# lastdancewithyou/multimodal_edema_prediction

Measured on AMD Instinct MI355X. Metric: multimodal train samples/sec, higher is better.
Workload: dtype bf16

## Files before the change

### include/medp_hip.h

```cpp
#ifndef MEDP_HIP_H
#define MEDP_HIP_H
#include <stddef.h>

#ifdef __cplusplus
extern "C" {
#endif

const char* medp_last_error(void);
int medp_version(void);
const char* medp_arch(void);

int medp_gemm_bf16_nt(const void* A, const void* W, void* C, int M, int N, int K, int lda, int ldw, int ldc,
                      const float* bias, const float* scale, const float* residual, int ldr, int act, int out_bf16,
                      void* stream);

size_t medp_gemm_nt_workspace_bytes(int M, int N, int K);
int medp_gemm_bf16_nt_ws(const void* A, const void* W, void* C, int M, int N, int K, int lda, int ldw, int ldc, const float* bias,
                         const float* scale, const float* residual, int ldr, int act, int out_bf16, float* workspace,
                         size_t workspace_bytes, void* stream);

int medp_gemm_f32_nt(const float* A, const float* W, float* C, int M, int N, int K, int lda, int ldw, int ldc, const float* bias,
                     const float* scale, const float* residual, int ldr, int act, void* stream);
int medp_gemm_f32_tn(const float* dY, const float* X, float* C, int M, int N, int K, int lddy, int ldx, void* stream);

// ... 65 lines not shown

int medp_cast_f32_bf16(const float* x, int ldx, void* y, int ldy, int rows, int cols, void* stream);
int medp_transpose_to_bf16(const void* x, int x_is_bf16, int ldx, void* y, int ldy, int rows, int cols, void* stream);
typedef struct {
    const void* src;
    void* dst_plain;
    void* dst_t;
    int rows, cols, ld_src, ld_plain, ld_t, reserved_;
} MedpOperandJob;
int medp_weight_operands_multi(const MedpOperandJob* dev_jobs, const int* dev_block_job, const int* dev_block_tile, int n_blocks,
                               void* stream);
int medp_gelu_bwd(const float* dy, const float* pre, float* dx, long long n, void* stream);
int medp_gelu_bf16_fwd(const void* pre, void* out, long long n, void* stream);
int medp_gelu_bf16_bwd(const void* dy, const void* pre, void* dx, long long n, void* stream);
int medp_im2col_patch(const float* pix, void* A, int B, int C, int H, int W, int patch, int kpad, void* stream);
int medp_vit_assemble(const float* patch, const float* cls, const float* pos, float* x, int B, int P, int D, void* stream);
int medp_pos_embed_bicubic(const float* pos, float* out, int src_side, int gh, int gw, int D, void* stream);
int medp_pos_embed_bicubic_bwd(const float* dout, float* dpos, int src_side, int gh, int gw, int D, void* stream);

typedef struct {
    const float *ln1_w, *ln1_b;
    const void* qkv_w;
    const float* qkv_b;
    const void* proj_w;
    const float *proj_b, *ls1;
    const float *ln2_w, *ln2_b;
    const void* fc1_w;
    const float* fc1_b;
    const void* fc2_w;
    const float *fc2_b, *ls2;
    const void *qkv_wg, *fc1_wg;
    const float *qkv_cs, *qkv_b2, *fc1_cs, *fc1_b2;
} MedpVitLayer;

typedef struct {
    int hidden, n_layers, n_heads, mlp_hidden, patch, pos_side, patch_kpad;
    float ln_eps;
    const void* patch_w;
    const float *patch_b, *cls, *pos;
    const float *final_ln_w, *final_ln_b;
    const MedpVitLayer* layers;
} MedpVitWeights;

size_t medp_vit_workspace_bytes(const MedpVitWeights* host_w, int B, int H, int W);
int medp_vit_forward(const MedpVitWeights* host_w, const float* pixels, int B, int H, int W, float* tokens_f32,
                     void* tokens_bf16, void* workspace, size_t workspace_bytes, void* stream);
int medp_vit_forward_part(const MedpVitWeights* w, const float* pixels, int B, int H, int W, float* tokens_f32, void* tokens_bf16,
                          void* workspace, size_t workspace_bytes, int first_layer, int last_layer, void* stream);

typedef struct {
    const float* g_attn;
    const void* qkv_w;
    const void* out_w;
    const float* g_ff;
    const void* ff1_w;
    const float* ff1_b;
    const void* ff2_w;
    const float* ff2_b;
    const float* g_final;
} MedpEncoderWeights;

typedef struct {
    int n_vars, n_static, d_embedding, n_heads, n_layers, d_ff, d_hidden_embed, d_hidden_tab, d_hidden_time, n_obs_rows,
// ... 193 lines not shown
```

### multimodal_edema_prediction_amd/abi.py

```python
from __future__ import annotations

import ctypes
import os
from ctypes import c_char_p, c_double, c_float, c_int, c_longlong, c_size_t, c_uint, c_void_p

import numpy as np
import torch

_HERE = os.path.dirname(os.path.abspath(__file__))
LIB_PATH = os.environ.get("MEDP_HIP_LIB") or os.path.join(_HERE, "libmedp_hip.so")

P, I, F, U, LL, SZ = c_void_p, c_int, c_float, c_uint, c_longlong, c_size_t


class MedpVitLayer(ctypes.Structure):
    _fields_ = [(n, P) for n in ("ln1_w", "ln1_b", "qkv_w", "qkv_b", "proj_w", "proj_b", "ls1", "ln2_w", "ln2_b",
                                 "fc1_w", "fc1_b", "fc2_w", "fc2_b", "ls2",
                                 "qkv_wg", "fc1_wg", "qkv_cs", "qkv_b2", "fc1_cs", "fc1_b2")]


class MedpVitWeights(ctypes.Structure):
    _fields_ = ([(n, I) for n in ("hidden", "n_layers", "n_heads", "mlp_hidden", "patch", "pos_side", "patch_kpad")]
                + [("ln_eps", F)]
                + [(n, P) for n in ("patch_w", "patch_b", "cls", "pos", "final_ln_w", "final_ln_b")]
                + [("layers", ctypes.POINTER(MedpVitLayer))])


class MedpEncoderWeights(ctypes.Structure):
    _fields_ = [(n, P) for n in ("g_attn", "qkv_w", "out_w", "g_ff", "ff1_w", "ff1_b", "ff2_w", "ff2_b", "g_final")]


class MedpDuettWeights(ctypes.Structure):
    _fields_ = ([(n, I) for n in ("n_vars", "n_static", "d_embedding", "n_heads", "n_layers", "d_ff", "d_hidden_embed",
                                  "d_hidden_tab", "d_hidden_time", "n_obs_rows", "final_norm")]
                + [("norm_eps", F)]
                + [(n, P) for n in ("emb_b4", "emb_l0", "emb_w4t", "n_obs_table",
                                    "tab_w0", "tab_b0", "tab_bn_scale", "tab_bn_shift", "tab_w4", "tab_b4", "special",
                                    "time_w0", "time_b0", "time_bn_scale", "time_bn_shift", "time_w3t", "time_b3",
                                    "rep_embedding", "event_embedding")]
                + [("event_enc", ctypes.POINTER(MedpEncoderWeights)), ("time_enc", ctypes.POINTER(MedpEncoderWeights))])


class MedpAdamTensor(ctypes.Structure):
    _fields_ = [("param", P), ("grad", P), ("exp_avg", P), ("exp_avg_sq", P), ("numel", LL), ("lr", F), ("weight_decay", F)]


class MedpOperandJob(ctypes.Structure):
    _fields_ = [("src", P), ("dst_plain", P), ("dst_t", P), ("rows", I), ("cols", I), ("ld_src", I), ("ld_plain", I), ("ld_t", I),
                ("reserved_", I)]


class MedpProbeProblem(ctypes.Structure):
    _fields_ = [("col_off", LL), ("row_off", LL), ("n_rows", I), ("F", I), ("y_col", I), ("j0", I), ("j1", I), ("reserved_", I)]


class MedpHeadProblem(ctypes.Structure):
    _fields_ = ([(n, P) for n in ("X", "Y", "M", "W", "b", "mW", "vW", "mb", "vb", "t", "perm", "loss_out")] + [("ldx", LL)]
                + [(n, I) for n in ("N", "ldy", "col0", "F", "L", "label_width", "bs", "S")]
                + [(n, c_double) for n in ("lr", "weight_decay", "beta1", "beta2", "eps")]
                + [("dropout_p", F), ("seed", U), ("stream_id", U), ("reserved_", I)])


SIGNATURES = {
    "medp_last_error": (c_char_p, []),
# ... 26 lines not shown
    "medp_attn_fq_split_bwd": (I, [P, I, P, I, P, P, I, LL, P, P, I, LL, P, I, P, P, I, LL, P, SZ, I, I, I, I, I, F, F, U, U, P]),
    "medp_layernorm_fwd": (I, [P, I, P, P, P, I, I, P, P, I, I, F, P]),
    "medp_colsum_workspace_bytes": (SZ, [I, I]),
    "medp_layernorm_bwd": (I, [P, I, P, I, P, P, P, P, I, I, P, P, P, I, I, P]),
    "medp_colsum_f32": (I, [P, I, P, P, I, I, P]),
    "medp_scalenorm_fwd": (I, [P, I, P, P, I, I, P, I, I, F, P]),
    "medp_scalenorm_bwd": (I, [P, I, P, I, P, P, P, I, I, P, P, I, I, P]),
    "medp_scalenorm_bwd_add": (I, [P, I, P, I, P, P, P, I, P, I, P, P, I, I, P]),
    "medp_cast_f32_bf16": (I, [P, I, P, I, I, I, P]),
    "medp_transpose_to_bf16": (I, [P, I, I, P, I, I, I, P]),
    "medp_weight_operands_multi": (I, [P, P, P, I, P]),
    "medp_gelu_bwd": (I, [P, P, P, LL, P]),
    "medp_gelu_bf16_fwd": (I, [P, P, LL, P]),
    "medp_gelu_bf16_bwd": (I, [P, P, P, LL, P]),
    "medp_im2col_patch": (I, [P, P, I, I, I, I, I, I, P]),
    "medp_vit_assemble": (I, [P, P, P, P, I, I, I, P]),
    "medp_pos_embed_bicubic": (I, [P, P, I, I, I, I, P]),
    "medp_pos_embed_bicubic_bwd": (I, [P, P, I, I, I, I, P]),
    "medp_vit_workspace_bytes": (SZ, [ctypes.POINTER(MedpVitWeights), I, I, I]),
    "medp_vit_forward": (I, [ctypes.POINTER(MedpVitWeights), P, I, I, I, P, P, P, SZ, P]),
    "medp_vit_forward_part": (I, [ctypes.POINTER(MedpVitWeights), P, I, I, I, P, P, P, SZ, I, I, P]),
    "medp_duett_embed_fwd": (I, [ctypes.POINTER(MedpDuettWeights), P, P, P, I, I, P, P, P, P, P, I, P]),
    "medp_duett_swap_add_norm": (I, [P, P, P, P, LL, P, F, P, P, I, I, I, I, P]),
    "medp_feats_to_input": (I, [P, P, LL, P, P, LL, P, I, P, P, P, P, I, I, I, I, I, F, F, U, U, P]),
    "medp_ssl_mask_batch": (I, [P, P, P, P, P, P, P, P, P, I, I, I, P]),
    "medp_duett_workspace_bytes": (SZ, [ctypes.POINTER(MedpDuettWeights), I, I]),
    "medp_duett_encode": (I, [ctypes.POINTER(MedpDuettWeights), P, P, P, I, I, P, P, P, P, SZ, P]),
    "medp_gelu_dropout_fwd": (I, [P, P, LL, F, U, U, P]),
    "medp_gelu_dropout_bwd": (I, [P, P, P, LL, F, U, U, P]),
    "medp_gelu_dropout_fwd_bf16": (I, [P, P, LL, F, U, U, P]),
    "medp_gelu_dropout_bwd_bf16": (I, [P, P, P, P, LL, F, U, U, P]),
    "medp_dropout_add": (I, [P, P, P, LL, F, U, U, P]),
    "medp_rowdot_fwd": (I, [P, I, P, P, P, I, I, P]),
    "medp_rowdot_bwd": (I, [P, P, I, P, P, P, P, I, I, P]),
    "medp_fusion_logits_fwd": (I, [P, P, P, P, P, P, P, P, P, P, I, I, P]),
    "medp_fusion_logits_bwd": (I, [P, P, P, P, P, P, P, P, P, P, P, P, I, I, P]),
# ... 110 lines not shown
```

### multimodal_edema_prediction_amd/csrc/elementwise.hip

```cpp
#include "common.h"
#include "medp_hip.h"

namespace {

__global__ __launch_bounds__(256) void cast_f32_bf16_kernel(const float* __restrict__ x, int ldx, bf16_t* __restrict__ y, int ldy,
                                                            int rows, int cols) {
    const int c4 = cols >> 2;
    const size_t total = (size_t)rows * c4;
    for (size_t i = (size_t)blockIdx.x * 256 + threadIdx.x; i < total; i += (size_t)gridDim.x * 256) {
        const int r = (int)(i / c4), c = (int)(i % c4) * 4;
        const float4 v = *(const float4*)(x + (size_t)r * ldx + c);
        uint2 o;
        o.x = pack_bf2(v.x, v.y);
        o.y = pack_bf2(v.z, v.w);
        *(uint2*)(y + (size_t)r * ldy + c) = o;
    }
}

template <typename TIN>
__global__ __launch_bounds__(256) void transpose_to_bf16_kernel(const TIN* __restrict__ x, int ldx, bf16_t* __restrict__ y, int ldy,
                                                                int rows, int cols) {
    __shared__ float tile[64][65];
    const int r0 = blockIdx.y * 64, c0 = blockIdx.x * 64;
    const int tx = threadIdx.x & 63, ty = threadIdx.x >> 6;
// ... 67 lines not shown
                                                            bf16_t* __restrict__ dx, size_t n8) {
    for (size_t i = (size_t)blockIdx.x * 256 + threadIdx.x; i < n8; i += (size_t)gridDim.x * 256) {
        const uint4 g = *(const uint4*)(dy + i * 8), p = *(const uint4*)(pre + i * 8);
        const uint32_t gw[4] = {g.x, g.y, g.z, g.w}, pw[4] = {p.x, p.y, p.z, p.w};
        uint32_t o[4];
#pragma unroll
        for (int k = 0; k < 4; ++k) {
            const float a = __uint_as_float(gw[k] << 16) * gelu_erf_grad(__uint_as_float(pw[k] << 16));
            const float b = __uint_as_float(gw[k] & 0xffff0000u) * gelu_erf_grad(__uint_as_float(pw[k] & 0xffff0000u));
            o[k] = pack_bf2(a, b);
        }
        *(uint4*)(dx + i * 8) = make_uint4(o[0], o[1], o[2], o[3]);
    }
}

__global__ __launch_bounds__(256) void im2col_patch_kernel(const float* __restrict__ pix, bf16_t* __restrict__ A, int B, int C, int H,
                                                           int W, int ps, int kpad) {
    const unsigned gh = H / ps, gw = W / ps, K = C * ps * ps, pp = ps * ps, k8 = kpad >> 3;
    const unsigned total = (unsigned)B * gh * gw * k8;
    for (unsigned i = blockIdx.x * 256u + threadIdx.x; i < total; i += gridDim.x * 256u) {
        const unsigned kc = i % k8, row = i / k8;
        const unsigned px = row % gw, r2 = row / gw, py = r2 % gh, b = r2 / gh;
        const float* img = pix + (size_t)b * C * H * W + (size_t)(py * ps) * W + px * ps;
        float v[8];
#pragma unroll
        for (int u = 0; u < 8; ++u) {
            const unsigned kk = kc * 8 + u;
            float x = 0.f;
            if (kk < K) {
                const unsigned c = kk / pp, rem = kk - c * pp, ii = rem / ps, jj = rem - ii * ps;
                x = img[((size_t)c * H + ii) * W + jj];
            }
// ... 133 lines not shown
extern "C" int medp_gelu_bf16_fwd(const void* pre, void* out, long long n, void* stream) {
    MEDP_CHECK_ARG(pre && out && n > 0 && n % 8 == 0, "gelu_bf16_fwd: bad argument (n must be a multiple of 8)");
    gelu_bf16_fwd_kernel<<<grid_for((size_t)n / 8), 256, 0, (hipStream_t)stream>>>((const bf16_t*)pre, (bf16_t*)out, (size_t)n / 8);
    MEDP_LAUNCH_CHECK("medp_gelu_bf16_fwd");
    return 0;
}

extern "C" int medp_gelu_bf16_bwd(const void* dy, const void* pre, void* dx, long long n, void* stream) {
    MEDP_CHECK_ARG(dy && pre && dx && n > 0 && n % 8 == 0, "gelu_bf16_bwd: bad argument (n must be a multiple of 8)");
    gelu_bf16_bwd_kernel<<<grid_for((size_t)n / 8), 256, 0, (hipStream_t)stream>>>((const bf16_t*)dy, (const bf16_t*)pre, (bf16_t*)dx,
                                                                                  (size_t)n / 8);
    MEDP_LAUNCH_CHECK("medp_gelu_bf16_bwd");
    return 0;
}

extern "C" int medp_im2col_patch(const float* pix, void* A, int B, int C, int H, int W, int patch, int kpad, void* stream) {
    MEDP_CHECK_ARG(pix && A && B > 0 && C > 0 && patch > 0, "im2col: bad argument");
    MEDP_CHECK_ARG(H >= patch && W >= patch, "im2col: image %dx%d smaller than the patch size %d", H, W, patch);
    MEDP_CHECK_ARG(kpad >= C * patch * patch && kpad % 8 == 0, "im2col: kpad must be >= C*p*p and a multiple of 8");
    const size_t total = (size_t)B * (H / patch) * (W / patch) * (kpad / 8);
    MEDP_CHECK_ARG(total < (1ull << 31), "im2col: B * patches * kpad / 8 must stay below 2^31");
    im2col_patch_kernel<<<grid_for(total), 256, 0, (hipStream_t)stream>>>(pix, (bf16_t*)A, B, C, H, W, patch, kpad);
    MEDP_LAUNCH_CHECK("medp_im2col_patch");
    return 0;
}

extern "C" int medp_vit_assemble(const float* patch, const float* cls, const float* pos, float* x, int B, int P, int D, void* stream) {
    MEDP_CHECK_ARG(patch && cls && pos && x && B > 0 && P > 0 && D % 4 == 0, "vit_assemble: bad argument");
    vit_assemble_kernel<<<grid_for((size_t)B * (P + 1) * D / 4), 256, 0, (hipStream_t)stream>>>(patch, cls, pos, x, B, P, D);
    MEDP_LAUNCH_CHECK("medp_vit_assemble");
    return 0;
}

extern "C" int medp_pos_embed_bicubic_bwd(const float* dout, float* dpos, int src_side, int gh, int gw, int D, void* stream) {
    MEDP_CHECK_ARG(dout && dpos && src_side > 0 && gh > 0 && gw > 0 && D > 0 && D % 4 == 0, "pos_embed_bicubic_bwd: bad argument");
    pos_bicubic_bwd_kernel<<<grid_for((size_t)(src_side * src_side + 1) * (D / 4)), 256, 0, (hipStream_t)stream>>>(dout, dpos, src_side, gh, gw, D);
    MEDP_LAUNCH_CHECK("medp_pos_embed_bicubic_bwd");
    return 0;
// ... 9 lines not shown
```

### multimodal_edema_prediction_amd/csrc/vit.hip

```cpp
#include "common.h"
#include "gemm_variants.h"
#include "medp_hip.h"

namespace {
inline size_t al(size_t x) { return (x + 255) & ~(size_t)255; }

struct VitWs {
    size_t a0, patch, pos, x, h, qkv, att, f, xb, stats, total;
};

template <int NT>
__global__ __launch_bounds__(256) void rowstats_cast_kernel(const float* __restrict__ x, bf16_t* __restrict__ xb, float* __restrict__ stats,
                                                            int M, int Mpad, int D) {
    const int lane = threadIdx.x & 63;
    const int row = blockIdx.x * 4 + (threadIdx.x >> 6);
    if (row >= Mpad) return;
    float s1[NT], s2[NT];
#pragma unroll
    for (int k = 0; k < NT; ++k) {
        s1[k] = s2[k] = 0.f;
        if (row < M) {
            const float4 v = *(const float4*)(x + (size_t)row * D + 4 * (lane + 64 * k));
            uint2 o;
            o.x = pack_bf2(v.x, v.y);
// ... 45 lines not shown
    return medp_gemm_run(MedpGemmArgs{A, W, C, M, N, K, K, K, N, bias, scale, residual, N, act, out_bf16, nullptr, 0, fold}, 1, nullptr, 0, stream);
}
}

extern "C" size_t medp_vit_workspace_bytes(const MedpVitWeights* w, int B, int H, int W) {
    if (!w || B <= 0 || H <= 0 || W <= 0 || w->patch <= 0) return 0;
    return plan(w, B, H, W).total;
}

extern "C" int medp_vit_forward(const MedpVitWeights* w, const float* pixels, int B, int H, int W, float* tokens_f32,
                                void* tokens_bf16, void* workspace, size_t workspace_bytes, void* stream) {
    MEDP_CHECK_ARG(w, "vit_forward: null argument");
    return medp_vit_forward_part(w, pixels, B, H, W, tokens_f32, tokens_bf16, workspace, workspace_bytes, 0, w->n_layers, stream);
}

extern "C" int medp_vit_forward_part(const MedpVitWeights* w, const float* pixels, int B, int H, int W, float* tokens_f32,
                                     void* tokens_bf16, void* workspace, size_t workspace_bytes, int first_layer, int last_layer,
                                     void* stream) {
    MEDP_CHECK_ARG(w && pixels && workspace, "vit_forward: null argument");
    MEDP_CHECK_ARG(0 <= first_layer && first_layer <= last_layer && last_layer <= w->n_layers,
                   "vit_forward: bad layer range [%d, %d) of %d", first_layer, last_layer, w->n_layers);
    const bool embed = first_layer == 0, finish = last_layer == w->n_layers;
    MEDP_CHECK_ARG(!finish || tokens_f32 || tokens_bf16, "vit_forward: no output requested");
    MEDP_CHECK_ARG(w->hidden == w->n_heads * 64, "vit_forward: head dim must be 64 (hidden %d, heads %d)", w->hidden, w->n_heads);
    MEDP_CHECK_ARG(H >= w->patch && W >= w->patch, "vit_forward: image %dx%d smaller than one patch (%d)", H, W, w->patch);
    const VitWs ws = plan(w, B, H, W);
    MEDP_CHECK_ARG(workspace_bytes >= ws.total, "vit_forward: workspace %zu < required %zu", workspace_bytes, ws.total);
    char* base = (char*)workspace;
    const int gh = H / w->patch, gw = W / w->patch, P = gh * gw, S = P + 1, M = B * S, D = w->hidden;
    void* a0 = base + ws.a0;
    float* patch = (float*)(base + ws.patch);
    float* pos = (float*)(base + ws.pos);
    float* x = (float*)(base + ws.x);
    void* h = base + ws.h;
    void* qkv = base + ws.qkv;
    void* att = base + ws.att;
    void* f = base + ws.f;

    if (embed) {
        MEDP_TRY(medp_im2col_patch(pixels, a0, B, 3, H, W, w->patch, w->patch_kpad, stream));
        MEDP_TRY(medp_gemm_bf16_nt(a0, w->patch_w, patch, B * P, D, w->patch_kpad, w->patch_kpad, w->patch_kpad, D, w->patch_b,
                                   nullptr, nullptr, 0, 0, 0, stream));
        const float* pos_used = w->pos;
        if (!(gh == w->pos_side && gw == w->pos_side)) {
            MEDP_TRY(medp_pos_embed_bicubic(w->pos, pos, w->pos_side, gh, gw, D, stream));
            pos_used = pos;
        }
        MEDP_TRY(medp_vit_assemble(patch, w->cls, pos_used, x, B, P, D, stream));
    }
    const float scale = 0.125f;
    if (fold_wanted(w, M) && first_layer < last_layer) {
        bf16_t* xb = (bf16_t*)(base + ws.xb);
        float* stats = (float*)(base + ws.stats);
        const int NT = D / 256, Mpad = (M + 255) / 256 * 256;
        hipStream_t st = (hipStream_t)stream;
        if (NT == 1) rowstats_cast_kernel<1><<<(Mpad + 3) / 4, 256, 0, st>>>(x, xb, stats, M, Mpad, D);
        else if (NT == 2) rowstats_cast_kernel<2><<<(Mpad + 3) / 4, 256, 0, st>>>(x, xb, stats, M, Mpad, D);
        else if (NT == 3) rowstats_cast_kernel<3><<<(Mpad + 3) / 4, 256, 0, st>>>(x, xb, stats, M, Mpad, D);
        else rowstats_cast_kernel<4><<<(Mpad + 3) / 4, 256, 0, st>>>(x, xb, stats, M, Mpad, D);
        MEDP_LAUNCH_CHECK("vit rowstats_cast");
        MedpGemmFold cons{}, prod{};
// ... 19 lines not shown
            MEDP_TRY(medp_attn_fwd_dh64(qkv, (const bf16_t*)qkv + D, (const bf16_t*)qkv + 2 * D, att, B, S, w->n_heads, 3 * D, 3 * D,
                                        3 * D, D, scale, stream));
            MEDP_TRY(block_gemm(att, L.proj_w, x, M, D, D, L.proj_b, L.ls1, x, 0, 0, plain, stream));
            MEDP_TRY(medp_layernorm_fwd(x, D, L.ln2_w, L.ln2_b, h, D, 1, nullptr, nullptr, M, D, w->ln_eps, stream));
            MEDP_TRY(block_gemm(h, L.fc1_w, f, M, w->mlp_hidden, D, L.fc1_b, nullptr, nullptr, 1, 1, plain, stream));
            MEDP_TRY(block_gemm(f, L.fc2_w, x, M, D, w->mlp_hidden, L.fc2_b, L.ls2, x, 0, 0, plain, stream));
        }
    }
    if (!finish) return 0;
    if (tokens_f32)
        MEDP_TRY(medp_layernorm_fwd(x, D, w->final_ln_w, w->final_ln_b, tokens_f32, D, 0, nullptr, nullptr, M, D, w->ln_eps, stream));
    if (tokens_bf16)
        MEDP_TRY(medp_layernorm_fwd(x, D, w->final_ln_w, w->final_ln_b, tokens_bf16, D, 1, nullptr, nullptr, M, D, w->ln_eps, stream));
    return 0;
}

extern "C" int medp_dbg_vit_lnfold(int on) {
    const int prev = g_vit_lnfold;
    g_vit_lnfold = on < 0 ? -1 : (on != 0);
    return prev;
}

extern "C" int medp_dbg_gemm_fold(const void* A, const void* W, void* C, int M, int N, int K, const float* bias, const float* scale,
                                  const float* residual, int act, int out_bf16, void* c2, float* stats_out, const float* stats_in,
                                  int stats_tiles, const float* colsum, float ln_eps, int ln_dim, void* stream) {
    MedpGemmFold f{};
    f.c2 = c2; f.ldc2 = N; f.stats_out = stats_out;
    f.stats_in = stats_in; f.stats_tiles = stats_tiles; f.colsum = colsum; f.ln_eps = ln_eps; f.ln_dim = ln_dim;
    MEDP_CHECK_ARG(medp_gemm_fold_eligible(M, N, K), "gemm(fold): M=%d N=%d K=%d does not take the 256-tile kernels", M, N, K);
    return block_gemm(A, W, C, M, N, K, bias, scale, residual, act, out_bf16, f, stream);
// ... 2 lines not shown
```

### multimodal_edema_prediction_amd/cxr.py

```python
from __future__ import annotations

import ctypes
from collections import namedtuple
from dataclasses import dataclass

import torch
import torch.nn as nn

from . import abi
from . import functional as Fn
from .abi import MedpVitLayer, MedpVitWeights, check, lib, ptr, stream


@dataclass
class Dinov2Cfg:
    hidden_size: int = 768
    num_hidden_layers: int = 12
    num_attention_heads: int = 12
    mlp_ratio: int = 4
    patch_size: int = 14
    image_size: int = 518
    layer_norm_eps: float = 1e-6
    layerscale_value: float = 1.0
    num_channels: int = 3
# ... 117 lines not shown
            for name, W, b, g, beta in (("qkv", qkv_w, qkv_b, blk.ln1_w, blk.ln1_b), ("fc1", blk.w1, blk.b1, blk.ln2_w, blk.ln2_b)):
                W32 = W.detach().to(torch.float32)
                wg = bf(W32 * g.detach().to(torch.float32)[None, :])
                setattr(L, name + "_wg", ptr(wg))
                setattr(L, name + "_cs", ptr(f32(wg.to(torch.float32).sum(dim=1))))
                setattr(L, name + "_b2", ptr(f32(b.detach().to(torch.float32) + W32 @ beta.detach().to(torch.float32))))
        w = MedpVitWeights()
        w.hidden, w.n_layers, w.n_heads, w.mlp_hidden = D, c.num_hidden_layers, c.num_attention_heads, D * c.mlp_ratio
        w.patch, w.pos_side, w.patch_kpad, w.ln_eps = c.patch_size, c.image_size // c.patch_size, pw.shape[1], c.layer_norm_eps
        w.patch_w = ptr(bf(pw))
        w.patch_b = ptr(f32(sd["embeddings.patch_embeddings.projection.bias"]))
        w.cls = ptr(f32(sd["embeddings.cls_token"].reshape(-1)))
        w.pos = ptr(f32(sd["embeddings.position_embeddings"].reshape(-1, D)))
        w.final_ln_w, w.final_ln_b = ptr(f32(sd["layernorm.weight"])), ptr(f32(sd["layernorm.bias"]))
        w.layers = ctypes.cast(layers, ctypes.POINTER(MedpVitLayer))
        self._prep, self._prep_key = (w, layers, keep), key
        return self._prep

    def forward(self, pixel_values: torch.Tensor, want_f32: bool = True, want_bf16: bool = False, layers=None, slot: int = 0, out16=None):
        abi.require_gpu()
        if pixel_values.dim() != 4 or pixel_values.shape[1] != self.cfg.num_channels:
            raise ValueError("Make sure that the channel dimension of the pixel values match with the one set in the "
                             f"configuration. Expected {self.cfg.num_channels} but got {tuple(pixel_values.shape)}.")
        if any(p.requires_grad for p in self.parameters()) and torch.is_grad_enabled():
            from .cxr_train import forward_training
            if out16 is not None:
                raise ValueError("out16 is a frozen-path argument (the training path returns fp32 tokens with a gradient)")
            tok = forward_training(self, pixel_values)
            return (tok if want_f32 else None), (tok if want_bf16 else None)
        if Fn.precision() == "fp32" and layers is None:
            from .cxr_train import forward_fp32
            tok = forward_fp32(self, pixel_values)
            t16 = None
            if want_bf16:
                t16 = tok.to(torch.bfloat16) if out16 is None else out16.copy_(tok)
            return (tok if want_f32 else None), t16
        w, _, _ = self._prepare()
        px = pixel_values.detach().to(torch.float32).contiguous()
        B, _, H, W = px.shape
        P = (H // self.cfg.patch_size) * (W // self.cfg.patch_size)
        need = lib().medp_vit_workspace_bytes(ctypes.byref(w), B, H, W)
        ws = self._ws.get(slot)
        if ws is None or ws.numel() < need or ws.device != px.device:
            ws = self._ws[slot] = torch.empty(need, dtype=torch.uint8, device=px.device)
        D = self.cfg.hidden_size
        first, last = (0, self.cfg.num_hidden_layers) if layers is None else layers
        fin = last == self.cfg.num_hidden_layers
        out32 = torch.empty((B, P + 1, D), dtype=torch.float32, device=px.device) if (want_f32 and fin) else None
        if out16 is not None:
            if out16.shape != (B, P + 1, D) or out16.dtype != torch.bfloat16 or not out16.is_contiguous() or out16.device != px.device:
                raise ValueError("out16 must be a contiguous bf16 [B, P+1, hidden] tensor on the input's device")
        else:
            out16 = torch.empty((B, P + 1, D), dtype=torch.bfloat16, device=px.device) if (want_bf16 and fin) else None
        check(lib().medp_vit_forward_part(ctypes.byref(w), ptr(px), B, H, W, ptr(out32), ptr(out16), ptr(ws), need, first, last,
                                          stream()), "vit_forward")
        return out32, out16


class CXREncoder(nn.Module):

    def __init__(self, model_name: str = "microsoft/rad-dino", freeze: bool = True, return_patches: bool = True, *,
                 config: Dinov2Cfg | None = None):
        super().__init__()
        self.backbone = Dinov2Backbone(config)
        if config is None and model_name and model_name != "synthetic":
            self._try_load_pretrained(model_name)
        self.d_out = self.backbone.cfg.hidden_size
        self.return_patches = return_patches
        if freeze:
            for p in self.backbone.parameters():
# ... 18 lines not shown
        return self

    def forward(self, pixel_values: torch.Tensor):
        tokens, _ = self.backbone(pixel_values)
        cls = tokens[:, 0]
        if self.return_patches:
            return cls, tokens[:, 1:]
        return cls

    def forward_bf16(self, pixel_values: torch.Tensor, slot: int = 0, out=None):
        if Fn.precision() == "fp32" and out is None and not (any(p.requires_grad for p in self.backbone.parameters()) and torch.is_grad_enabled()):
            return self.backbone(pixel_values, want_f32=True, want_bf16=False)[0]
        _, t16 = self.backbone(pixel_values, want_f32=False, want_bf16=True, slot=slot, out16=out)
        return t16

    def forward_bf16_part(self, pixel_values: torch.Tensor, first: int, last: int):
        if any(p.requires_grad for p in self.backbone.parameters()):
            raise RuntimeError("the encoder can only be run in pieces when it is frozen")
        _, t16 = self.backbone(pixel_values, want_f32=False, want_bf16=True, layers=(first, last))
        return t16
```

### multimodal_edema_prediction_amd/graph_step.py

```python
from __future__ import annotations

import os

import torch

from . import autograd_ops as _A, dp, engine
from .streams import new_stream, note_capture_origin
from .abi import check, lib, ptr, stream


def _stacked(v):
    return v if torch.is_tensor(v) else torch.stack(tuple(v))


class _TrainSnapshot:

    def __init__(self, modules, epoch, params=(), optimizer=None, extra=()):
        self.params, self.opt, self.modules, self.epoch = list(params), optimizer, list(modules), epoch
        with torch.no_grad():
            self.p = [q.detach().clone() for q in self.params]
            self.bufs = [(m, n, b.detach().clone()) for m in self.modules for n, b in m.named_buffers()]
            self.extra = [(t, t.detach().clone()) for t in extra]
            self.epoch0 = epoch.detach().clone()
            if optimizer is not None:
                self.state = {id(q): {k: (v.detach().clone() if torch.is_tensor(v) else v) for k, v in optimizer.state.get(q, {}).items()}
                              for q in self.params}
                self.host_step = optimizer._step
# ... 102 lines not shown

    def _replay(self):
        self._check_frozen_unchanged()
        self.opt.refresh_lrs()
        self.g.replay()
        self._after_replay()
        return self.out

    def _after_replay(self):
        self.opt.note_external_step()


class _PipelinedStep(_CapturedStep):

    def _setup(self, optimizer, device, world, group, split, pipeline, warmup, before_capture, after_capture=None):
        self.world, self.group = world, group
        self.pipeline = bool(pipeline)
        self.split = bool(split) or world > 1
        self.arena = None
        self.force_collective = False
        self._pool = None
        self._expect = None
        self._staged, self.stage = None, None
        self.frozen_stream = new_stream(device) if self.pipeline else None
        self._build(optimizer, device, warmup, before_capture)
        if after_capture is not None:
            after_capture()
        self.phase_log = None
        if self.pipeline and os.environ.get("MEDP_PHASE_CHECK", "0") == "1":
            penalty, t_copy = self._staging_penalty()
            self.phase_log = (len(self._pad_streams), round(penalty * 1e3, 3), round(t_copy * 1e3, 3))

    def _streams_before_capture(self):
        self._pad_streams = [new_stream(self.device, raw=True) for _ in range(int(os.environ.get("MEDP_PRE_CAPTURE_STREAMS", str(self._default_pad_streams()))))]
        self.copy_stream = new_stream(self.device)

    def _default_pad_streams(self) -> int:
        return 3
# ... 5 lines not shown
            self.arena = dp.FlatGradArena(self.params, used=used, group=self.group)
            self.arena.bind(zero=True)
            snap.restore()
        self._zero_grads()
        self._advance()
        if last and os.environ.get("MEDP_OPERAND_POOL", "1") == "1":
            with _A.record_operands() as log:
                self._whole_fwd_bwd()
            self._pool = _A.WeightOperandPool(log, self.device)
        else:
            self._whole_fwd_bwd()
        self._allreduce()
        self.opt.step()

    def _captured_step(self):
        if not self.split:
            self._advance()
            return self._whole_fwd_bwd(then=self.opt.step)
        self.arena.flat.zero_()
        self._advance()
        return self._whole_fwd_bwd()

    def _staging_penalty(self, n: int = 6):
        import time
        dev_b, host_b = self._calib_batches()
        snap = _TrainSnapshot(self._stateful_modules(), self.epoch, self.params, self.opt, extra=self._handover_tensors())
        expect = self._expect

        def timed(pool, staged):
            ts = []
# ... 28 lines not shown
    def _zero_grads(self):
        if self.arena is None:
            self.opt.zero_grad(set_to_none=True)
        else:
            self.arena.bind(zero=True)

    def _advance(self):
        self._advance_epoch()
        if self._pool is not None:
            self._pool.refresh()

    def _allreduce(self):
        if self.arena is not None and (self.world > 1 or self.force_collective):
            self.arena.all_reduce(force=self.force_collective)

    def _whole_fwd_bwd(self, then=None):
        if not self.pipeline:
            out = self._train_fwd_bwd()
            if then is not None:
                then()
            return out
        cur = torch.cuda.current_stream(self.device)
        self.frozen_stream.wait_stream(cur)
        with torch.cuda.stream(self.frozen_stream):
            self._frozen_forward()
        out = self._train_fwd_bwd()
        if then is not None:
            then()
        cur.wait_stream(self.frozen_stream)
        self._hand_over()
        return out

    def _after_replay(self):
        if not self.split:
            return super()._after_replay()
        ring = self._split_events()
        ring[0].record()
        self._allreduce()
        ring[1].record()
        self.opt.relaunch()
# ... 21 lines not shown
        if self.stage is None:
            self.stage = {k: torch.empty_like(v) for k, v in self._stage_buffers().items()}
            self.h2d_done, self.stage_free = torch.cuda.Event(), torch.cuda.Event()
            self.stage_free.record(torch.cuda.current_stream(self.device))
        with torch.cuda.stream(self.copy_stream):
            self.copy_stream.wait_event(self.stage_free)
            self._stage_h2d(next_batch, after_next)
            self.h2d_done.record(self.copy_stream)
        self._staged = (next_batch, after_next)

    def step(self, batch: dict | None = None, next_batch: dict | None = None, after_next: dict | None = None) -> dict:
        st = self._staged
        staged = self.pipeline and batch is not None and next_batch is not None and st is not None and st[0] is batch and st[1] is next_batch
        if batch is not None and self.pipeline and self._expect is not batch:
            self.prime(batch)
        if staged:
            cur = torch.cuda.current_stream(self.device)
            cur.wait_event(self.h2d_done)
            self._take_staged()
            self.stage_free.record(cur)
            self._expect = next_batch
        else:
            if batch is not None:
                self.load_batch(batch)
            nb = next_batch if next_batch is not None else batch
            if self.pipeline and nb is not None:
                self._load_next(nb)
                self._expect = nb
        if self.pipeline and after_next is not None and next_batch is not None and not next_batch["pixel_values"].is_cuda:
            self._stage(next_batch, after_next)
        else:
            self._staged = None
        return self._replay()


class GraphedTeacherStep(_PipelinedStep):
    def __init__(self, teacher, loss_fn, optimizer, example_batch: dict, device, world: int = 1, group=None, warmup: int = 3,
                 split: bool = False, before_capture=None, pipeline_cxr: bool = False, after_capture=None):
        self.teacher, self.loss_fn = teacher, loss_fn
        b = engine._move_lists(example_batch, device)
        self.x_ts = torch.stack(b["x_ts"]).contiguous()
        self.x_static = torch.stack(b["x_static"]).contiguous()
        self.bin_ends = torch.stack(b["bin_ends"]).contiguous()
        self.pixels = b["pixel_values"].clone()
        if pipeline_cxr:
            if any(p.requires_grad for p in teacher.cxr.parameters()):
                raise ValueError("pipeline_cxr needs a frozen CXR encoder")
            self.pixels_next = self.pixels.clone()
            with torch.no_grad():
                self.tok_cur = teacher.cxr.forward_bf16(self.pixels).clone()
            self.tok_next = torch.empty_like(self.tok_cur)
        self.y_multi = b["y_multi"].clone().float()
        self.y_mask = b["y_multi_mask"].clone().float()
        engine._set_train_with_frozen_eval(teacher)
        self._setup(optimizer, device, world, group, split, pipeline_cxr, warmup, before_capture, after_capture)

    def _frozen_forward(self):
        with torch.no_grad():
            self.teacher.cxr.forward_bf16(self.pixels_next, out=self.tok_next)

    def _stateful_modules(self):
        return [self.teacher]

    def _handover_tensors(self):
        return [self.tok_cur] if self.pipeline else []

    def _small_buffers(self):
        return {"x_ts": self.x_ts, "x_static": self.x_static, "bin_ends": self.bin_ends, "y_multi": self.y_multi, "y_multi_mask": self.y_mask}

    def _calib_batches(self):
        d = {k: v.clone() for k, v in dict(self._small_buffers(), pixel_values=self.pixels).items()}
        h = {k: v.cpu().pin_memory() for k, v in d.items()}
        return [dict(d), dict(d)], [dict(h), dict(h)]

    def _hand_over(self):
        self.tok_cur.copy_(self.tok_next)

    def _train_fwd_bwd(self):
        B = self.x_ts.shape[0]
        out = self.teacher(tuple(self.x_ts[i] for i in range(B)), tuple(self.x_static[i] for i in range(B)),
                           tuple(self.bin_ends[i] for i in range(B)), self.pixels,
                           **({"_cxr_tokens16": self.tok_cur} if self.pipeline else {}))
        losses = self.loss_fn(out["img_logits"], out["ts_logits"], out["fusion_logits"], self.y_multi, self.y_mask)
        losses["total"].backward()
        return {"loss": losses["total"].detach(), "img_total": losses["img_total"], "ts_total": losses["ts_total"],
                "fus_total": losses["fus_total"], "fusion_logits": out["fusion_logits"].detach(), "main_logit": out["main_logit"].detach()}

    def prime(self, batch: dict) -> None:
        with torch.no_grad():
            self.tok_cur.copy_(self.teacher.cxr.forward_bf16(batch["pixel_values"].to(self.device, non_blocking=True)))
        self._expect = batch
# ... 45 lines not shown
        self._setup(optimizer, device, world, group, split, pipeline_teacher, warmup, before_capture, after_capture)

    def _default_pad_streams(self) -> int:
        return 1 if self.swap_roles else 3

    def _teacher_logit(self, bufs, forked: bool = False):
        B = bufs["x_ts"].shape[0]
        kw = {"_overlap": False} if (forked and "_overlap" in self._teacher_kw) else {}
        return self.teacher(tuple(bufs["x_ts"][i] for i in range(B)), tuple(bufs["x_static"][i] for i in range(B)),
                            tuple(bufs["bin_ends"][i] for i in range(B)), bufs["pixel_values"], **kw)["main_logit"]

    def _frozen_forward(self):
        with torch.no_grad():
            self.z_next = self._teacher_logit(self.nxt, forked=not self.swap_roles)

    def _whole_fwd_bwd(self, then=None):
        if not (self.pipeline and self.swap_roles):
            return super()._whole_fwd_bwd(then)
        cur = torch.cuda.current_stream(self.device)
        ts = self.frozen_stream
        ts.wait_stream(cur)
        with torch.cuda.stream(ts):
            out = self._train_fwd_bwd()
            if then is not None:
                then()
        self._frozen_forward()
        cur.wait_stream(ts)
        self._hand_over()
        return out

# ... 110 lines not shown
```

Measured before the change: 13250.

## Gather batch inputs via device pointer table and fork frozen encoder earlier

Adds a device-side pointer table so the captured graph reads batch tensors in place: the frozen ViT im2col reads pixels through a slot pointer and a gather kernel copies the small inputs, which replaces per-step host loads and copies. The frozen encoder forward is forked at the start of the captured step. Its blocks run on the side stream and the final layernorm writes straight into tok_cur at hand-over, which drops the tok_next copy. The interpolated position-embedding grid is cached to skip the bicubic kernel. This adds complexity, pinned ring-buffer synchronisation, and risks stale pointers if the table update races with graph replay.

```diff
diff --git a/include/medp_hip.h b/include/medp_hip.h
--- a/include/medp_hip.h
+++ b/include/medp_hip.h
@@ -103,6 +103,14 @@
 int medp_gelu_bf16_fwd(const void* pre, void* out, long long n, void* stream);
 int medp_gelu_bf16_bwd(const void* dy, const void* pre, void* dx, long long n, void* stream);
 int medp_im2col_patch(const float* pix, void* A, int B, int C, int H, int W, int patch, int kpad, void* stream);
+int medp_im2col_patch_slot(const float* const* pix_slot, void* A, int B, int C, int H, int W, int patch, int kpad, void* stream);
+#define MEDP_GATHER_MAX_JOBS 8
+typedef struct {
+    int slot, reserved_;
+    void* dst;
+    long long bytes;
+} MedpGatherJob;
+int medp_gather_inputs(const void* const* table, int n_slots, const MedpGatherJob* jobs, int n, void* stream);
 int medp_vit_assemble(const float* patch, const float* cls, const float* pos, float* x, int B, int P, int D, void* stream);
 int medp_pos_embed_bicubic(const float* pos, float* out, int src_side, int gh, int gw, int D, void* stream);
 int medp_pos_embed_bicubic_bwd(const float* dout, float* dpos, int src_side, int gh, int gw, int D, void* stream);
@@ -129,6 +137,8 @@
     const float *patch_b, *cls, *pos;
     const float *final_ln_w, *final_ln_b;
     const MedpVitLayer* layers;
+    const float* pos_grid;
+    int pos_grid_h, pos_grid_w;
 } MedpVitWeights;
 
 size_t medp_vit_workspace_bytes(const MedpVitWeights* host_w, int B, int H, int W);
@@ -136,6 +146,8 @@
                      void* tokens_bf16, void* workspace, size_t workspace_bytes, void* stream);
 int medp_vit_forward_part(const MedpVitWeights* w, const float* pixels, int B, int H, int W, float* tokens_f32, void* tokens_bf16,
                           void* workspace, size_t workspace_bytes, int first_layer, int last_layer, void* stream);
+int medp_vit_forward_part_slot(const MedpVitWeights* w, const float* const* pixels_slot, int B, int H, int W, float* tokens_f32,
+                               void* tokens_bf16, void* workspace, size_t workspace_bytes, int first_layer, int last_layer, void* stream);
 
 typedef struct {
     const float* g_attn;
diff --git a/multimodal_edema_prediction_amd/abi.py b/multimodal_edema_prediction_amd/abi.py
--- a/multimodal_edema_prediction_amd/abi.py
+++ b/multimodal_edema_prediction_amd/abi.py
@@ -23,7 +23,8 @@
     _fields_ = ([(n, I) for n in ("hidden", "n_layers", "n_heads", "mlp_hidden", "patch", "pos_side", "patch_kpad")]
                 + [("ln_eps", F)]
                 + [(n, P) for n in ("patch_w", "patch_b", "cls", "pos", "final_ln_w", "final_ln_b")]
-                + [("layers", ctypes.POINTER(MedpVitLayer))])
+                + [("layers", ctypes.POINTER(MedpVitLayer))]
+                + [("pos_grid", P), ("pos_grid_h", I), ("pos_grid_w", I)])
 
 
 class MedpEncoderWeights(ctypes.Structure):
@@ -48,6 +49,10 @@
 class MedpOperandJob(ctypes.Structure):
     _fields_ = [("src", P), ("dst_plain", P), ("dst_t", P), ("rows", I), ("cols", I), ("ld_src", I), ("ld_plain", I), ("ld_t", I),
                 ("reserved_", I)]
+
+
+class MedpGatherJob(ctypes.Structure):
+    _fields_ = [("slot", I), ("reserved_", I), ("dst", P), ("bytes", LL)]
 
 
 class MedpProbeProblem(ctypes.Structure):
@@ -104,12 +109,15 @@
     "medp_gelu_bf16_fwd": (I, [P, P, LL, P]),
     "medp_gelu_bf16_bwd": (I, [P, P, P, LL, P]),
     "medp_im2col_patch": (I, [P, P, I, I, I, I, I, I, P]),
+    "medp_im2col_patch_slot": (I, [P, P, I, I, I, I, I, I, P]),
+    "medp_gather_inputs": (I, [P, I, ctypes.POINTER(MedpGatherJob), I, P]),
     "medp_vit_assemble": (I, [P, P, P, P, I, I, I, P]),
     "medp_pos_embed_bicubic": (I, [P, P, I, I, I, I, P]),
     "medp_pos_embed_bicubic_bwd": (I, [P, P, I, I, I, I, P]),
     "medp_vit_workspace_bytes": (SZ, [ctypes.POINTER(MedpVitWeights), I, I, I]),
     "medp_vit_forward": (I, [ctypes.POINTER(MedpVitWeights), P, I, I, I, P, P, P, SZ, P]),
     "medp_vit_forward_part": (I, [ctypes.POINTER(MedpVitWeights), P, I, I, I, P, P, P, SZ, I, I, P]),
+    "medp_vit_forward_part_slot": (I, [ctypes.POINTER(MedpVitWeights), P, I, I, I, P, P, P, SZ, I, I, P]),
     "medp_duett_embed_fwd": (I, [ctypes.POINTER(MedpDuettWeights), P, P, P, I, I, P, P, P, P, P, I, P]),
     "medp_duett_swap_add_norm": (I, [P, P, P, P, LL, P, F, P, P, I, I, I, I, P]),
     "medp_feats_to_input": (I, [P, P, LL, P, P, LL, P, I, P, P, P, P, I, I, I, I, I, F, F, U, U, P]),
diff --git a/multimodal_edema_prediction_amd/csrc/elementwise.hip b/multimodal_edema_prediction_amd/csrc/elementwise.hip
--- a/multimodal_edema_prediction_amd/csrc/elementwise.hip
+++ b/multimodal_edema_prediction_amd/csrc/elementwise.hip
@@ -105,8 +105,9 @@
     }
 }
 
-__global__ __launch_bounds__(256) void im2col_patch_kernel(const float* __restrict__ pix, bf16_t* __restrict__ A, int B, int C, int H,
-                                                           int W, int ps, int kpad) {
+__global__ __launch_bounds__(256) void im2col_patch_kernel(const float* pix_arg, const float* const* __restrict__ pix_slot,
+                                                           bf16_t* __restrict__ A, int B, int C, int H, int W, int ps, int kpad) {
+    const float* __restrict__ pix = pix_slot ? *pix_slot : pix_arg;
     const unsigned gh = H / ps, gw = W / ps, K = C * ps * ps, pp = ps * ps, k8 = kpad >> 3;
     const unsigned total = (unsigned)B * gh * gw * k8;
     for (unsigned i = blockIdx.x * 256u + threadIdx.x; i < total; i += gridDim.x * 256u) {
@@ -270,14 +271,60 @@
     return 0;
 }
 
-extern "C" int medp_im2col_patch(const float* pix, void* A, int B, int C, int H, int W, int patch, int kpad, void* stream) {
-    MEDP_CHECK_ARG(pix && A && B > 0 && C > 0 && patch > 0, "im2col: bad argument");
+namespace {
+int im2col_patch(const float* pix, const float* const* pix_slot, void* A, int B, int C, int H, int W, int patch, int kpad, void* stream) {
+    MEDP_CHECK_ARG((pix || pix_slot) && A && B > 0 && C > 0 && patch > 0, "im2col: bad argument");
     MEDP_CHECK_ARG(H >= patch && W >= patch, "im2col: image %dx%d smaller than the patch size %d", H, W, patch);
     MEDP_CHECK_ARG(kpad >= C * patch * patch && kpad % 8 == 0, "im2col: kpad must be >= C*p*p and a multiple of 8");
     const size_t total = (size_t)B * (H / patch) * (W / patch) * (kpad / 8);
     MEDP_CHECK_ARG(total < (1ull << 31), "im2col: B * patches * kpad / 8 must stay below 2^31");
-    im2col_patch_kernel<<<grid_for(total), 256, 0, (hipStream_t)stream>>>(pix, (bf16_t*)A, B, C, H, W, patch, kpad);
+    im2col_patch_kernel<<<grid_for(total), 256, 0, (hipStream_t)stream>>>(pix, pix_slot, (bf16_t*)A, B, C, H, W, patch, kpad);
     MEDP_LAUNCH_CHECK("medp_im2col_patch");
+    return 0;
+}
+
+struct GatherJobs {
+    MedpGatherJob j[MEDP_GATHER_MAX_JOBS];
+};
+__global__ __launch_bounds__(256) void gather_inputs_kernel(const void* const* __restrict__ table, GatherJobs jobs) {
+    const MedpGatherJob j = jobs.j[blockIdx.y];
+    const char* src = (const char*)table[j.slot];
+    char* dst = (char*)j.dst;
+    if (src == dst) return;
+    const size_t bytes = (size_t)j.bytes, first = (size_t)blockIdx.x * 256 + threadIdx.x, step = (size_t)gridDim.x * 256;
+    if ((((size_t)src | (size_t)dst | bytes) & 15) == 0) {
+        for (size_t i = first; i < (bytes >> 4); i += step) ((uint4*)dst)[i] = ((const uint4*)src)[i];
+    } else {
+        for (size_t i = first; i < (bytes >> 2); i += step) ((unsigned*)dst)[i] = ((const unsigned*)src)[i];
+    }
+}
+}
+
+extern "C" int medp_im2col_patch(const float* pix, void* A, int B, int C, int H, int W, int patch, int kpad, void* stream) {
+    MEDP_CHECK_ARG(pix, "im2col: bad argument");
+    return im2col_patch(pix, nullptr, A, B, C, H, W, patch, kpad, stream);
+}
+
+extern "C" int medp_im2col_patch_slot(const float* const* pix_slot, void* A, int B, int C, int H, int W, int patch, int kpad, void* stream) {
+    MEDP_CHECK_ARG(pix_slot, "im2col: bad argument");
+    return im2col_patch(nullptr, pix_slot, A, B, C, H, W, patch, kpad, stream);
+}
+
+extern "C" int medp_gather_inputs(const void* const* table, int n_slots, const MedpGatherJob* jobs, int n, void* stream) {
+    MEDP_CHECK_ARG(table && jobs && n_slots > 0 && n > 0 && n <= MEDP_GATHER_MAX_JOBS, "gather_inputs: bad argument (1 .. %d jobs)",
+                   MEDP_GATHER_MAX_JOBS);
+    GatherJobs g{};
+    long long most = 0;
+    for (int i = 0; i < n; ++i) {
+        const MedpGatherJob& j = jobs[i];
+        MEDP_CHECK_ARG(j.slot >= 0 && j.slot < n_slots && j.dst && j.bytes > 0 && j.bytes % 4 == 0 && ((size_t)j.dst & 3) == 0,
+                       "gather_inputs: job %d: slot %d of %d, %lld bytes (dword-aligned destination and size)", i, j.slot, n_slots, j.bytes);
+        g.j[i] = j;
+        most = j.bytes > most ? j.bytes : most;
+    }
+    const size_t wgs = ((size_t)most / 16 + 255) / 256;
+    gather_inputs_kernel<<<dim3((unsigned)(wgs < 1 ? 1 : (wgs > 256 ? 256 : wgs)), n), 256, 0, (hipStream_t)stream>>>(table, g);
+    MEDP_LAUNCH_CHECK("medp_gather_inputs");
     return 0;
 }
 
diff --git a/multimodal_edema_prediction_amd/csrc/vit.hip b/multimodal_edema_prediction_amd/csrc/vit.hip
--- a/multimodal_edema_prediction_amd/csrc/vit.hip
+++ b/multimodal_edema_prediction_amd/csrc/vit.hip
@@ -83,14 +83,15 @@
     return medp_vit_forward_part(w, pixels, B, H, W, tokens_f32, tokens_bf16, workspace, workspace_bytes, 0, w->n_layers, stream);
 }
 
-extern "C" int medp_vit_forward_part(const MedpVitWeights* w, const float* pixels, int B, int H, int W, float* tokens_f32,
-                                     void* tokens_bf16, void* workspace, size_t workspace_bytes, int first_layer, int last_layer,
-                                     void* stream) {
-    MEDP_CHECK_ARG(w && pixels && workspace, "vit_forward: null argument");
+namespace {
+int vit_forward_part(const MedpVitWeights* w, const float* pixels, const float* const* pixels_slot, int B, int H, int W, float* tokens_f32,
+                     void* tokens_bf16, void* workspace, size_t workspace_bytes, int first_layer, int last_layer, void* stream) {
+    MEDP_CHECK_ARG(w && workspace, "vit_forward: null argument");
     MEDP_CHECK_ARG(0 <= first_layer && first_layer <= last_layer && last_layer <= w->n_layers,
                    "vit_forward: bad layer range [%d, %d) of %d", first_layer, last_layer, w->n_layers);
-    const bool embed = first_layer == 0, finish = last_layer == w->n_layers;
-    MEDP_CHECK_ARG(!finish || tokens_f32 || tokens_bf16, "vit_forward: no output requested");
+    const bool embed = first_layer == 0, finish = last_layer == w->n_layers && (tokens_f32 || tokens_bf16);
+    MEDP_CHECK_ARG(finish || embed || first_layer < last_layer, "vit_forward: no output requested");
+    MEDP_CHECK_ARG(!embed || pixels || pixels_slot, "vit_forward: null argument");
     MEDP_CHECK_ARG(w->hidden == w->n_heads * 64, "vit_forward: head dim must be 64 (hidden %d, heads %d)", w->hidden, w->n_heads);
     MEDP_CHECK_ARG(H >= w->patch && W >= w->patch, "vit_forward: image %dx%d smaller than one patch (%d)", H, W, w->patch);
     const VitWs ws = plan(w, B, H, W);
@@ -107,13 +108,18 @@
     void* f = base + ws.f;
 
     if (embed) {
-        MEDP_TRY(medp_im2col_patch(pixels, a0, B, 3, H, W, w->patch, w->patch_kpad, stream));
+        if (pixels) MEDP_TRY(medp_im2col_patch(pixels, a0, B, 3, H, W, w->patch, w->patch_kpad, stream));
+        else MEDP_TRY(medp_im2col_patch_slot(pixels_slot, a0, B, 3, H, W, w->patch, w->patch_kpad, stream));
         MEDP_TRY(medp_gemm_bf16_nt(a0, w->patch_w, patch, B * P, D, w->patch_kpad, w->patch_kpad, w->patch_kpad, D, w->patch_b,
                                    nullptr, nullptr, 0, 0, 0, stream));
         const float* pos_used = w->pos;
         if (!(gh == w->pos_side && gw == w->pos_side)) {
-            MEDP_TRY(medp_pos_embed_bicubic(w->pos, pos, w->pos_side, gh, gw, D, stream));
-            pos_used = pos;
+            if (w->pos_grid && w->pos_grid_h == gh && w->pos_grid_w == gw) {
+                pos_used = w->pos_grid;
+            } else {
+                MEDP_TRY(medp_pos_embed_bicubic(w->pos, pos, w->pos_side, gh, gw, D, stream));
+                pos_used = pos;
+            }
         }
         MEDP_TRY(medp_vit_assemble(patch, w->cls, pos_used, x, B, P, D, stream));
     }
@@ -163,6 +169,20 @@
         MEDP_TRY(medp_layernorm_fwd(x, D, w->final_ln_w, w->final_ln_b, tokens_bf16, D, 1, nullptr, nullptr, M, D, w->ln_eps, stream));
     return 0;
 }
+}
+
+extern "C" int medp_vit_forward_part(const MedpVitWeights* w, const float* pixels, int B, int H, int W, float* tokens_f32,
+                                     void* tokens_bf16, void* workspace, size_t workspace_bytes, int first_layer, int last_layer,
+                                     void* stream) {
+    return vit_forward_part(w, pixels, nullptr, B, H, W, tokens_f32, tokens_bf16, workspace, workspace_bytes, first_layer, last_layer, stream);
+}
+
+extern "C" int medp_vit_forward_part_slot(const MedpVitWeights* w, const float* const* pixels_slot, int B, int H, int W, float* tokens_f32,
+                                          void* tokens_bf16, void* workspace, size_t workspace_bytes, int first_layer, int last_layer,
+                                          void* stream) {
+    return vit_forward_part(w, nullptr, pixels_slot, B, H, W, tokens_f32, tokens_bf16, workspace, workspace_bytes, first_layer, last_layer,
+                            stream);
+}
 
 extern "C" int medp_dbg_vit_lnfold(int on) {
     const int prev = g_vit_lnfold;
diff --git a/multimodal_edema_prediction_amd/cxr.py b/multimodal_edema_prediction_amd/cxr.py
--- a/multimodal_edema_prediction_amd/cxr.py
+++ b/multimodal_edema_prediction_amd/cxr.py
@@ -155,10 +155,27 @@
         w.pos = ptr(f32(sd["embeddings.position_embeddings"].reshape(-1, D)))
         w.final_ln_w, w.final_ln_b = ptr(f32(sd["layernorm.weight"])), ptr(f32(sd["layernorm.bias"]))
         w.layers = ctypes.cast(layers, ctypes.POINTER(MedpVitLayer))
-        self._prep, self._prep_key = (w, layers, keep), key
+        self._prep, self._prep_key = (w, layers, keep, {}), key
         return self._prep
 
-    def forward(self, pixel_values: torch.Tensor, want_f32: bool = True, want_bf16: bool = False, layers=None, slot: int = 0, out16=None):
+    def _pos_grid(self, gh: int, gw: int):
+        w, _, keep, tabs = self._prepare()
+        if not getattr(self, "cache_pos_grid", True) or (gh == w.pos_side and gw == w.pos_side):
+            return None
+        t = tabs.get((gh, gw))
+        if t is None:
+            if torch.cuda.is_current_stream_capturing():
+                return None
+            dev = next(self.parameters()).device
+            t = torch.empty((1 + gh * gw, w.hidden), dtype=torch.float32, device=dev)
+            check(lib().medp_pos_embed_bicubic(w.pos, ptr(t), w.pos_side, gh, gw, w.hidden, stream()), "pos_embed_bicubic")
+            torch.cuda.current_stream(dev).synchronize()
+            tabs[(gh, gw)] = t
+            keep.append(t)
+        return t
+
+    def forward(self, pixel_values: torch.Tensor, want_f32: bool = True, want_bf16: bool = False, layers=None, slot: int = 0, out16=None,
+                finish: bool = True, pixels_slot: int | None = None):
         abi.require_gpu()
         if pixel_values.dim() != 4 or pixel_values.shape[1] != self.cfg.num_channels:
             raise ValueError("Make sure that the channel dimension of the pixel values match with the one set in the "
@@ -176,9 +193,11 @@
             if want_bf16:
                 t16 = tok.to(torch.bfloat16) if out16 is None else out16.copy_(tok)
             return (tok if want_f32 else None), t16
-        w, _, _ = self._prepare()
+        w = self._prepare()[0]
         px = pixel_values.detach().to(torch.float32).contiguous()
         B, _, H, W = px.shape
+        pos = self._pos_grid(H // self.cfg.patch_size, W // self.cfg.patch_size)
+        w.pos_grid, w.pos_grid_h, w.pos_grid_w = ptr(pos), H // self.cfg.patch_size, W // self.cfg.patch_size
         P = (H // self.cfg.patch_size) * (W // self.cfg.patch_size)
         need = lib().medp_vit_workspace_bytes(ctypes.byref(w), B, H, W)
         ws = self._ws.get(slot)
@@ -186,15 +205,19 @@
             ws = self._ws[slot] = torch.empty(need, dtype=torch.uint8, device=px.device)
         D = self.cfg.hidden_size
         first, last = (0, self.cfg.num_hidden_layers) if layers is None else layers
-        fin = last == self.cfg.num_hidden_layers
+        fin = last == self.cfg.num_hidden_layers and finish
         out32 = torch.empty((B, P + 1, D), dtype=torch.float32, device=px.device) if (want_f32 and fin) else None
         if out16 is not None:
             if out16.shape != (B, P + 1, D) or out16.dtype != torch.bfloat16 or not out16.is_contiguous() or out16.device != px.device:
                 raise ValueError("out16 must be a contiguous bf16 [B, P+1, hidden] tensor on the input's device")
         else:
             out16 = torch.empty((B, P + 1, D), dtype=torch.bfloat16, device=px.device) if (want_bf16 and fin) else None
-        check(lib().medp_vit_forward_part(ctypes.byref(w), ptr(px), B, H, W, ptr(out32), ptr(out16), ptr(ws), need, first, last,
-                                          stream()), "vit_forward")
+        if pixels_slot is not None:
+            check(lib().medp_vit_forward_part_slot(ctypes.byref(w), pixels_slot, B, H, W, ptr(out32), ptr(out16), ptr(ws), need, first, last,
+                                                   stream()), "vit_forward")
+        else:
+            check(lib().medp_vit_forward_part(ctypes.byref(w), ptr(px), B, H, W, ptr(out32), ptr(out16), ptr(ws), need, first, last,
+                                              stream()), "vit_forward")
         return out32, out16
 
 
@@ -243,6 +266,16 @@
         _, t16 = self.backbone(pixel_values, want_f32=False, want_bf16=True, slot=slot, out16=out)
         return t16
 
+    def forward_blocks(self, pixel_values: torch.Tensor, slot: int = 0, pixels_slot: int | None = None) -> None:
+        if any(p.requires_grad for p in self.backbone.parameters()):
+            raise RuntimeError("the encoder can only be run in pieces when it is frozen")
+        self.backbone(pixel_values, want_f32=False, want_bf16=False, layers=(0, self.backbone.cfg.num_hidden_layers), slot=slot, finish=False,
+                      pixels_slot=pixels_slot)
+
+    def finish_bf16(self, pixel_values: torch.Tensor, out: torch.Tensor, slot: int = 0) -> torch.Tensor:
+        n = self.backbone.cfg.num_hidden_layers
+        return self.backbone(pixel_values, want_f32=False, want_bf16=True, layers=(n, n), slot=slot, out16=out)[1]
+
     def forward_bf16_part(self, pixel_values: torch.Tensor, first: int, last: int):
         if any(p.requires_grad for p in self.backbone.parameters()):
             raise RuntimeError("the encoder can only be run in pieces when it is frozen")
diff --git a/multimodal_edema_prediction_amd/graph_step.py b/multimodal_edema_prediction_amd/graph_step.py
--- a/multimodal_edema_prediction_amd/graph_step.py
+++ b/multimodal_edema_prediction_amd/graph_step.py
@@ -6,11 +6,44 @@
 
 from . import autograd_ops as _A, dp, engine
 from .streams import new_stream, note_capture_origin
-from .abi import check, lib, ptr, stream
+from .abi import MedpGatherJob, check, lib, ptr, stream
 
 
 def _stacked(v):
     return v if torch.is_tensor(v) else torch.stack(tuple(v))
+
+
+class _BatchTable:
+    RING = 16
+
+    def __init__(self, statics, device):
+        self.statics, self.device = list(statics), device
+        self.now = [t.data_ptr() for t in self.statics]
+        self.dev = torch.tensor(self.now, dtype=torch.int64, device=device)
+        self.ring = torch.zeros((self.RING, len(self.statics)), dtype=torch.int64).pin_memory()
+        self.copied = [None] * self.RING
+        self.row = 0
+        self.held = self.held_before = None
+
+    def slot(self, i: int) -> int:
+        return self.dev.data_ptr() + 8 * i
+
+    def point_at(self, tensors=None):
+        tensors = [None] * len(self.statics) if tensors is None else list(tensors)
+        ptrs = [(s if t is None else t).data_ptr() for s, t in zip(self.statics, tensors)]
+        self.held_before, self.held = self.held, tensors
+        if ptrs == self.now:
+            return
+        r = self.row
+        self.row = (r + 1) % self.RING
+        if self.copied[r] is None:
+            self.copied[r] = torch.cuda.Event()
+        else:
+            self.copied[r].synchronize()
+        self.ring[r].copy_(torch.tensor(ptrs, dtype=torch.int64))
+        self.dev.copy_(self.ring[r], non_blocking=True)
+        self.copied[r].record(torch.cuda.current_stream(self.device))
+        self.now = ptrs
 
 
 class _TrainSnapshot:
@@ -143,14 +176,17 @@
 class _PipelinedStep(_CapturedStep):
 
     def _setup(self, optimizer, device, world, group, split, pipeline, warmup, before_capture, after_capture=None):
-        self.world, self.group = world, group
+        self.world, self.group, self.device = world, group, device
         self.pipeline = bool(pipeline)
+        self.encoder_path = os.environ.get("MEDP_ENCODER_PATH", "1") != "0"
+        self.table = self._make_batch_table() if (self.pipeline and self.encoder_path) else None
         self.split = bool(split) or world > 1
         self.arena = None
         self.force_collective = False
         self._pool = None
         self._expect = None
         self._staged, self.stage = None, None
+        self._forked = False
         self.frozen_stream = new_stream(device) if self.pipeline else None
         self._build(optimizer, device, warmup, before_capture)
         if after_capture is not None:
@@ -186,6 +222,9 @@
         self.opt.step()
 
     def _captured_step(self):
+        if self.encoder_path:
+            self._fork_frozen()
+            self._gather_inputs()
         if not self.split:
             self._advance()
             return self._whole_fwd_bwd(then=self.opt.step)
@@ -244,6 +283,26 @@
         if self.arena is not None and (self.world > 1 or self.force_collective):
             self.arena.all_reduce(force=self.force_collective)
 
+    def _make_batch_table(self):
+        return None
+
+    def _gather_inputs(self):
+        pass
+
+    def _table_sources(self, batch: dict, next_batch: dict):
+        return None
+
+    def _forks_frozen(self) -> bool:
+        return self.pipeline
+
+    def _fork_frozen(self):
+        if not self._forks_frozen() or self._forked:
+            return
+        self.frozen_stream.wait_stream(torch.cuda.current_stream(self.device))
+        with torch.cuda.stream(self.frozen_stream):
+            self._frozen_forward()
+        self._forked = True
+
     def _whole_fwd_bwd(self, then=None):
         if not self.pipeline:
             out = self._train_fwd_bwd()
@@ -251,9 +310,8 @@
                 then()
             return out
         cur = torch.cuda.current_stream(self.device)
-        self.frozen_stream.wait_stream(cur)
-        with torch.cuda.stream(self.frozen_stream):
-            self._frozen_forward()
+        self._fork_frozen()
+        self._forked = False
         out = self._train_fwd_bwd()
         if then is not None:
             then()
@@ -305,7 +363,12 @@
         staged = self.pipeline and batch is not None and next_batch is not None and st is not None and st[0] is batch and st[1] is next_batch
         if batch is not None and self.pipeline and self._expect is not batch:
             self.prime(batch)
-        if staged:
+        nb = next_batch if next_batch is not None else batch
+        named = self._table_sources(batch, nb) if (self.table is not None and not staged and batch is not None) else None
+        if named is not None:
+            self.table.point_at(named)
+            self._expect = nb
+        elif staged:
             cur = torch.cuda.current_stream(self.device)
             cur.wait_event(self.h2d_done)
             self._take_staged()
@@ -314,10 +377,11 @@
         else:
             if batch is not None:
                 self.load_batch(batch)
-            nb = next_batch if next_batch is not None else batch
             if self.pipeline and nb is not None:
                 self._load_next(nb)
                 self._expect = nb
+        if named is None and self.table is not None:
+            self.table.point_at(None)
         if self.pipeline and after_next is not None and next_batch is not None and not next_batch["pixel_values"].is_cuda:
             self._stage(next_batch, after_next)
         else:
@@ -340,7 +404,7 @@
             self.pixels_next = self.pixels.clone()
             with torch.no_grad():
                 self.tok_cur = teacher.cxr.forward_bf16(self.pixels).clone()
-            self.tok_next = torch.empty_like(self.tok_cur)
+            self.tok_next = None
         self.y_multi = b["y_multi"].clone().float()
         self.y_mask = b["y_multi_mask"].clone().float()
         engine._set_train_with_frozen_eval(teacher)
@@ -348,6 +412,11 @@
 
     def _frozen_forward(self):
         with torch.no_grad():
+            if self.encoder_path:
+                self.teacher.cxr.forward_blocks(self.pixels_next, pixels_slot=None if self.table is None else self.table.slot(0))
+                return
+            if self.tok_next is None:
+                self.tok_next = torch.empty_like(self.tok_cur)
             self.teacher.cxr.forward_bf16(self.pixels_next, out=self.tok_next)
 
     def _stateful_modules(self):
@@ -358,6 +427,25 @@
 
     def _small_buffers(self):
         return {"x_ts": self.x_ts, "x_static": self.x_static, "bin_ends": self.bin_ends, "y_multi": self.y_multi, "y_multi_mask": self.y_mask}
+
+    def _make_batch_table(self):
+        return _BatchTable([self.pixels_next] + list(self._small_buffers().values()), self.device)
+
+    def _gather_inputs(self):
+        if self.table is None:
+            return
+        bufs = list(self._small_buffers().values())
+        jobs = (MedpGatherJob * len(bufs))()
+        for i, buf in enumerate(bufs):
+            jobs[i].slot, jobs[i].dst, jobs[i].bytes = 1 + i, ptr(buf), buf.numel() * buf.element_size()
+        check(lib().medp_gather_inputs(ptr(self.table.dev), 1 + len(bufs), jobs, len(bufs), stream()), "gather_inputs")
+
+    def _table_sources(self, batch: dict, next_batch: dict):
+        src = [next_batch["pixel_values"]] + [batch[k] for k in self._small_buffers()]
+        for t, buf in zip(src, self.table.statics):
+            if not (torch.is_tensor(t) and t.device == buf.device and t.dtype == buf.dtype and t.shape == buf.shape and t.is_contiguous()):
+                return None
+        return src
 
     def _calib_batches(self):
         d = {k: v.clone() for k, v in dict(self._small_buffers(), pixel_values=self.pixels).items()}
@@ -365,7 +453,11 @@
         return [dict(d), dict(d)], [dict(h), dict(h)]
 
     def _hand_over(self):
-        self.tok_cur.copy_(self.tok_next)
+        if self.encoder_path:
+            with torch.no_grad():
+                self.teacher.cxr.finish_bf16(self.pixels_next, self.tok_cur)
+        else:
+            self.tok_cur.copy_(self.tok_next)
 
     def _train_fwd_bwd(self):
         B = self.x_ts.shape[0]
@@ -441,6 +533,9 @@
         with torch.no_grad():
             self.z_next = self._teacher_logit(self.nxt, forked=not self.swap_roles)
 
+    def _forks_frozen(self) -> bool:
+        return self.pipeline and not self.swap_roles
+
     def _whole_fwd_bwd(self, then=None):
         if not (self.pipeline and self.swap_roles):
             return super()._whole_fwd_bwd(then)
```

Result: no change. 13290, median of 5 (+0.3%).
